# shamim-hussain/tgt

Hardware: AMD Instinct MI355X
Metric: graphs/sec training step, TGT-At 24L PCQM batch 256, 1/2/4/8 MI355X (higher is better)
Workload: dtype bf16

## Files before the change

tgt_amd/csrc/triplet_attention_proj.hip:

```cpp
#include <cstdlib>
#include "triplet_common.hpp"

namespace tgt {

namespace proj2 {
constexpr int kC = xtile::kC, kKS = 16, kRowBytes = xtile::kRowBytes, kSlots = kRowBytes / 16;
constexpr int kXPitch = xtile::kPitch;
constexpr int kXTile = 64 * kXPitch;
constexpr int kSlab = 32 * 8 * 16 * 2;
constexpr int kOffSets = 2 * kXTile, kSet = 3 * kSlab;
constexpr int kOffO = kOffSets + 2 * kSet, kOffBias = kOffO + 2 * kSlab;
constexpr int kLds = kOffBias + 8 * 48 * 4;
constexpr uint32_t kNone = 0xffffffffu;
__device__ __forceinline__ int xoff(int row, int slot) { return xtile::off(row, slot); }
}

__device__ __forceinline__ void zero_o_rows(__amdgpu_buffer_rsrc_t r_out, int tid, int N, uint32_t o_row, uint32_t o_base, uint32_t o_j, int j0) {
    const int srow = (tid & 511) >> 4, sslot = tid & 15;
    const uint32_t vo = (srow < N && tid >= 512) ? (uint32_t)srow * o_row + o_base + (uint32_t)sslot * 16u : proj2::kNone;
    for (int j = j0; j < N; ++j) {
        u32x4_t z = {0, 0, 0, 0};
        __builtin_amdgcn_raw_buffer_store_b128(z, r_out, (int)vo, (int)((uint32_t)j * o_j), TGT_ST_AUX);
    }
}

template <typename T, int DIR, bool STORE, bool RG>
__device__ __forceinline__ void proj2_walk(const tgt_triplet_attention_args& a, const int32_t* node_counts, const TriCtx& c,
                                           const T* x, const T* w, char* smem, int tid) {
    using namespace proj2;
    constexpr int D = 16, HG = 8;
    using G = TriGeo<T, D, HG>;
    using F = frag_t<T>;
    const int lane = tid & 63, wave = tid >> 6, r = lane & 31, hi = lane >> 5;
#ifdef TGT_PROBES
    const uint32_t ablate = a._pad1;
#else
    constexpr uint32_t ablate = 0;
#endif
    const bool attend = wave < 8;
    const int hw = wave & 7;
    const int N = c.N;
    char* xbuf = smem;
    char* sets = smem + kOffSets;
    char* oslab = smem + kOffO;
    const float* bias_w = reinterpret_cast<const float*>(smem + kOffBias) + hw * 48;

    const int64_t sz = sizeof(T), Nl = N;
    const __amdgpu_buffer_rsrc_t r_x = graph_rsrc(x, Nl * Nl * kRowBytes, c.b);
    const uint32_t hch = (uint32_t)(c.g * HG * D * sz), lds_ = (uint32_t)(a.ld_qkv[DIR] * sz), ldo_ = (uint32_t)(a.ld_out * sz);
    const __amdgpu_buffer_rsrc_t r_dst = graph_rsrc(a.qkv[DIR], Nl * Nl * a.ld_qkv[DIR] * sz, c.b);
    const __amdgpu_buffer_rsrc_t r_out = graph_rsrc(a.out, Nl * Nl * a.ld_out * sz, c.b);
    const uint32_t q_row = (uint32_t)N * lds_, q_j = lds_;
    const uint32_t kv_row = DIR == 0 ? lds_ : (uint32_t)N * lds_, kv_j = DIR == 0 ? (uint32_t)N * lds_ : lds_;
    const uint32_t o_row = (uint32_t)N * ldo_, o_j = ldo_;
    auto store_step = [&](int jq, bool qkv_live, int jo, bool o_live) {
        int t_ = tid;
        asm volatile("" : "+v"(t_));
        const int srow = (t_ & 511) >> 4, sslot = t_ & 15, shalf = t_ >> 9;
        const int s_lds = G::lds_off(srow, sslot);
        const bool row_ok = srow < N;
        const uint32_t c16 = (uint32_t)sslot * 16u + hch;
        if constexpr (!STORE) {
            const uint4 vb = *reinterpret_cast<const uint4*>(oslab + (jo & 1) * kSlab + s_lds);
            const uint32_t vo_o = (uint32_t)srow * o_row + (uint32_t)jo * o_j + (uint32_t)(a.o_off[DIR] * sz) + c16;
            u32x4_t db = {vb.x, vb.y, vb.z, vb.w};
            if (ablate & 2) return;
            __builtin_amdgcn_sched_barrier(0);
            __builtin_amdgcn_raw_buffer_store_b128(db, r_out, (int)((row_ok && o_live && shalf == 1) ? vo_o : kNone), 0, TGT_ST_AUX);
            __builtin_amdgcn_sched_barrier(0);
            return;
        }
        const char* set = sets + (jq & 1) * kSet;
        const uint4 va = *reinterpret_cast<const uint4*>(set + shalf * kSlab + s_lds);
        const uint4 vb = *reinterpret_cast<const uint4*>((shalf == 0 ? set + 2 * kSlab : oslab + (jo & 1) * kSlab) + s_lds);
        const uint32_t vo_a = (uint32_t)srow * (shalf == 0 ? q_row : kv_row) + (uint32_t)jq * (shalf == 0 ? q_j : kv_j) +
                              (uint32_t)((shalf == 0 ? a.q_off[DIR] : a.k_off[DIR]) * sz) + c16;
        const uint32_t vo_v = (uint32_t)srow * kv_row + (uint32_t)jq * kv_j + (uint32_t)(a.v_off[DIR] * sz) + c16;
        const uint32_t vo_o = (uint32_t)srow * o_row + (uint32_t)jo * o_j + (uint32_t)(a.o_off[DIR] * sz) + c16;
        u32x4_t da = {va.x, va.y, va.z, va.w}, db = {vb.x, vb.y, vb.z, vb.w};
        if (ablate & 2) return;
        __builtin_amdgcn_sched_barrier(0);
        __builtin_amdgcn_raw_buffer_store_b128(da, r_dst, (int)((row_ok && qkv_live) ? vo_a : kNone), 0, TGT_ST_AUX);
        __builtin_amdgcn_raw_buffer_store_b128(db, r_dst, (int)((row_ok && qkv_live && shalf == 0) ? vo_v : kNone), 0, TGT_ST_AUX);
        __builtin_amdgcn_raw_buffer_store_b128(db, r_out, (int)((row_ok && o_live && shalf == 1) ? vo_o : kNone), 0, TGT_ST_AUX);
        __builtin_amdgcn_sched_barrier(0);
    };

    const int n = tri_node_count<RG>(node_counts, c.b, N);
    if ((a.graph_scale && a.graph_scale[c.b] == 0.f) || (RG && n == 0)) {
        zero_o_rows(r_out, tid, N, o_row, (uint32_t)(a.o_off[DIR] * sz) + hch, o_j, 0);
        return;
    }

    const int l16 = lane & 15, l4 = lane >> 4;
#ifndef TGT_PROJ_PRIO
#define TGT_PROJ_PRIO 1
#endif
    if (TGT_PROJ_PRIO != 0 && __builtin_amdgcn_readfirstlane(wave) >= 8 == (TGT_PROJ_PRIO == 1)) __builtin_amdgcn_s_setprio(1);
    if (attend) {
        float biasM[16], gate[16];
        const ThirdArm ta = tri_third_arm(a, DIR);
        arm_stage_load<T, HG, 1>(ta, c.b, DIR, c.g, N, 0, smem, tid);
        __syncthreads();
        arm_stage_read<T, HG, 1, false>(ta, smem, DIR, hw, N, r, hi, 0, 0, biasM, gate);
        __syncthreads();
        constexpr int kXIt = DIR == 0 ? 4 : 2;
        uint32_t xvo[kXIt];
        int xlo[kXIt];
#pragma unroll
        for (int it = 0; it < kXIt; ++it) {
            const int cidx = it * 512 + tid, row = cidx >> 5, slot = cidx & 31;
            const int node = row & 31;
            xvo[it] = node < N ? (row < 32 ? (uint32_t)node * (uint32_t)N * kRowBytes : (uint32_t)node * kRowBytes) + (uint32_t)slot * 16u : kNone;
            xlo[it] = xoff(row, slot);
        }
        uint4 px[kXIt];
        auto x_issue = [&](int jx) {
            const bool live = jx < n && !(ablate & 1);
#pragma unroll
            for (int it = 0; it < kXIt; ++it) {
                const bool kvrows = DIR == 0 && it >= 2;
                const uint32_t so = live ? (uint32_t)jx * (kvrows ? (uint32_t)N * kRowBytes : (uint32_t)kRowBytes) : 0u;
                const u32x4_t v = __builtin_amdgcn_raw_buffer_load_b128(r_x, (int)(live ? xvo[it] : kNone), (int)so, 0);
                px[it] = make_uint4(v.x, v.y, v.z, v.w);
            }
        };
        auto x_commit = [&](int jx) {
            char* xt = xbuf + (jx & 1) * kXTile;
#pragma unroll
            for (int it = 0; it < kXIt; ++it) *reinterpret_cast<uint4*>(xt + xlo[it]) = px[it];
        };
        F ident_d[1];
        make_ident_d<T, 1>(ident_d, r, hi);
        x_issue(0);
        x_commit(0);
        x_issue(1);
        x_commit(1);
        __syncthreads();
        __syncthreads();
        if constexpr (STORE) store_step(0, true, 0, false);
        for (int j = 0; j < n; ++j) {
            x_issue(j + 2);
            asm volatile("" ::: "memory");
            if (!(ablate & 8)) {
                const char* set = sets + (j & 1) * kSet;
                F fq[1], fk[1], fv[1];
                read_frags<T, D, HG>(fq, set, hw, r, hi);
                read_frags<T, D, HG>(fk, set + kSlab, hw, r, hi);
                read_frags<T, D, HG>(fv, set + 2 * kSlab, hw, r, hi);
                f32x16 z0 = {0}, z1 = {0};
                f32x16 st = mma32(fk[0], fq[0], z0);
                f32x16 vt = mma32(fv[0], ident_d[0], z1);
                float mx = -INFINITY;
#pragma unroll
                for (int q = 0; q < 16; ++q) {
                    st[q] = st[q] * a.scale + biasM[q];
                    mx = fmaxf(mx, st[q]);
                }
                mx = fmaxf(mx, xhalf(mx));
                float sum = 0.f;
#pragma unroll
                for (int q = 0; q < 16; ++q) {
                    st[q] = fast_exp(st[q] - mx);
                    sum += st[q];
                }
                sum += xhalf(sum);
                const float inv = fast_rcp(sum);
#pragma unroll
                for (int q = 0; q < 16; ++q) st[q] = st[q] * inv * gate[q];
                f32x16 o = {0};
#pragma unroll
                for (int cc = 0; cc < 2; ++cc) o = mma32(pack_chunk<T>(vt, cc), pack_chunk<T>(st, cc), o);
                write_rows<T, D, HG>(oslab + (j & 1) * kSlab, o, hw, r, hi);
            }
            x_commit(j + 2);
            __syncthreads();
            if constexpr (STORE) store_step(j + 1, j + 1 < n, j, true);
        }
    } else {
        F wq[kKS / 2], wkv[kKS];
        {
            const T* rq = w + (int64_t)(a.q_off[DIR] + c.h * D + l16) * kC;
            const T* rkv = w + (int64_t)((r < 16 ? a.k_off[DIR] : a.v_off[DIR]) + c.h * D + (r & 15)) * kC;
#pragma unroll
            for (int s2 = 0; s2 < kKS / 2; ++s2) wq[s2] = load_frag<T>(rq + 32 * s2 + 8 * l4);
#pragma unroll
            for (int s2 = 0; s2 < kKS; ++s2) wkv[s2] = load_frag<T>(rkv + 16 * s2 + 8 * hi);
        }
        auto project = [&](int jn) {
            const char* xt = xbuf + (jn & 1) * kXTile;
            char* set = sets + (jn & 1) * kSet;
            constexpr int kv0 = DIR == 0 ? 32 : 0;
            {
                f32x16 kva;
#pragma unroll
                for (int q = 0; q < 16; ++q) kva[q] = bias_w[16 + acc_row(q, hi)];
#pragma unroll
                for (int s2 = 0; s2 < kKS; ++s2) {
                    const F xk = load_frag<T>(reinterpret_cast<const T*>(xt + xoff(kv0 + r, 2 * s2 + hi)));
                    kva = mma32(wkv[s2], xk, kva);
                    if ((s2 & 3) == 3) __builtin_amdgcn_sched_barrier(0);
                }
#pragma unroll
                for (int part = 0; part < 2; ++part)
#pragma unroll
                    for (int q = 0; q < 2; ++q) {
                        T tmp[4];
#pragma unroll
                        for (int t = 0; t < 4; ++t) tmp[t] = from_f32<T>(kva[8 * part + 4 * q + t]);
                        uint2 v;
                        __builtin_memcpy(&v, tmp, 8);
                        *reinterpret_cast<uint2*>(set + (1 + part) * kSlab + G::lds_elem(r, hw * D + 8 * q + 4 * hi)) = v;
                    }
            }
            __builtin_amdgcn_sched_barrier(0);
            {
                f32x4 q0, q1;
#pragma unroll
                for (int t = 0; t < 4; ++t) q0[t] = q1[t] = bias_w[4 * l4 + t];
#pragma unroll
                for (int s2 = 0; s2 < kKS / 2; ++s2) {
                    const F x0 = load_frag<T>(reinterpret_cast<const T*>(xt + xoff(l16, 4 * s2 + l4)));
                    const F x1 = load_frag<T>(reinterpret_cast<const T*>(xt + xoff(16 + l16, 4 * s2 + l4)));
                    q0 = mma16x32(wq[s2], x0, q0);
                    q1 = mma16x32(wq[s2], x1, q1);
                    if (s2 & 1) __builtin_amdgcn_sched_barrier(0);
                }
                T t0[4], t1[4];
#pragma unroll
                for (int t = 0; t < 4; ++t) { t0[t] = from_f32<T>(q0[t]); t1[t] = from_f32<T>(q1[t]); }
                uint2 v0, v1;
                __builtin_memcpy(&v0, t0, 8);
                __builtin_memcpy(&v1, t1, 8);
                *reinterpret_cast<uint2*>(set + G::lds_elem(l16, hw * D + 4 * l4)) = v0;
                *reinterpret_cast<uint2*>(set + G::lds_elem(16 + l16, hw * D + 4 * l4)) = v1;
            }
        };
        __syncthreads();
        __syncthreads();
        __syncthreads();
        project(0);
        __syncthreads();
        if constexpr (STORE) store_step(0, true, 0, false);
        for (int j = 0; j < n; ++j) {
            if (j + 1 < n && !(ablate & 4)) project(j + 1);
            __syncthreads();
            store_step(j + 1, j + 1 < n, j, true);
        }
    }
    if constexpr (RG) {
        int t_ = tid;
        asm volatile("" : "+v"(t_));
        zero_o_rows(r_out, t_, N, o_row, (uint32_t)(a.o_off[DIR] * sz) + hch, o_j, n);
    }
}

template <typename T, bool STORE, typename... NC>
__global__ void __launch_bounds__(1024, 4) tri_att_proj_fwd_kernel(const tgt_triplet_attention_args a, const T* x, const T* w, const T* bias,
                                                                   NC... nc) {
    constexpr bool RG = sizeof...(NC) > 0;
    const int32_t* node_counts = tri_counts_ptr(nc...);
    constexpr int D = 16, HG = 8;
    extern __shared__ __attribute__((aligned(16))) char smem[];
    const int tid = threadIdx.x, lane = tid & 63, wave = tid >> 6;
    const TriCtx c = tri_ctx<T, D, HG>(a, wave & 7);
    const int dir = c.dir;
    if (wave >= 8 && lane < 48) {
        const int part = lane >> 4, d = lane & 15;
        const int off = part == 0 ? a.q_off[dir] : (part == 1 ? a.k_off[dir] : a.v_off[dir]);
        reinterpret_cast<float*>(smem + proj2::kOffBias)[(wave & 7) * 48 + lane] = to_f32(bias[off + c.h * D + d]);
    }
    if (dir == 0) proj2_walk<T, 0, STORE, RG>(a, node_counts, c, x, w, smem, tid);
    else proj2_walk<T, 1, STORE, RG>(a, node_counts, c, x, w, smem, tid);
}

template <typename T>
static int launch_proj(const tgt_triplet_attention_args& a, const int32_t* nc, const void* x, const void* w, const void* bias, hipStream_t st) {
    const int grid = a.B * 2 * (a.H / 8);
    static_assert(ArmStage<T, 8, 1>::kBytes <= proj2::kOffO, "arm stage must fit the aliased area");
#ifdef TGT_PROBES
    static const int ablate = getenv("TGT_PROJ_ABLATE") ? atoi(getenv("TGT_PROJ_ABLATE")) : 0;
    tgt_triplet_attention_args aa = a;
    aa._pad1 = (uint32_t)ablate;
#else
    const tgt_triplet_attention_args& aa = a;
#endif
    const T *xp = reinterpret_cast<const T*>(x), *wp = reinterpret_cast<const T*>(w), *bp = reinterpret_cast<const T*>(bias);
    const dim3 g(grid), blk(1024);
    if (a.flags & TGT_TRI_NO_QKV_STORE)
        return nc ? launch_lds<tri_att_proj_fwd_kernel<T, false, const int32_t*>>("tri_att_proj_fwd_kernel", g, blk, proj2::kLds, st, aa, xp, wp, bp, nc)
                  : launch_lds<tri_att_proj_fwd_kernel<T, false>>("tri_att_proj_fwd_kernel", g, blk, proj2::kLds, st, aa, xp, wp, bp);
    return nc ? launch_lds<tri_att_proj_fwd_kernel<T, true, const int32_t*>>("tri_att_proj_fwd_kernel", g, blk, proj2::kLds, st, aa, xp, wp, bp, nc)
              : launch_lds<tri_att_proj_fwd_kernel<T, true>>("tri_att_proj_fwd_kernel", g, blk, proj2::kLds, st, aa, xp, wp, bp);
}

int triplet_attention_proj_supported(const tgt_triplet_attention_args* a, int C) {
    return a && a->dropout_p == 0.f && a->N <= 32 && a->D == 16 && a->H % 8 == 0 && (a->dtype == TGT_BF16 || a->dtype == TGT_F16) &&
           C == 256;
}

int triplet_attention_proj_run(const tgt_triplet_attention_args* a, const int32_t* nc, const void* x, int C, const void* w,
                               const void* bias, hipStream_t st) {
    if (!a || !x || !w || !bias) return set_error(TGT_ERR_INVALID, "projected triplet attention: null argument");
    if (a->B < 0 || a->N < 0 || a->H <= 0) return set_error(TGT_ERR_INVALID, "projected triplet attention: bad sizes");
    if (a->B == 0 || a->N == 0) return TGT_OK;
    if (!triplet_attention_proj_supported(a, C))
        return set_error(TGT_ERR_UNSUPPORTED,
                         "projected triplet attention needs N <= 32, D = 16, H %% 8 == 0, a 16-bit dtype, C = 256 and no attention dropout "
                         "(got N=%d D=%d H=%d dtype=%d C=%d)", a->N, a->D, a->H, a->dtype, C);
    const bool store = !(a->flags & TGT_TRI_NO_QKV_STORE);
    for (int dir = 0; dir < 2; ++dir) {
        if ((store && !a->qkv[dir]) || !a->out || !a->mask) return set_error(TGT_ERR_INVALID, "projected triplet attention: null tensor");
        if (store && ((a->ld_qkv[dir] * 2) % 16 || (a->q_off[dir] * 2) % 16 || (a->k_off[dir] * 2) % 16 || (a->v_off[dir] * 2) % 16 ||
                      ((uintptr_t)a->qkv[dir] % 16)))
            return set_error(TGT_ERR_INVALID, "projected triplet attention: rows/offsets must be 16-byte aligned");
        if ((a->ld_out * 2) % 16 || (a->o_off[dir] * 2) % 16 || ((uintptr_t)a->out % 16))
            return set_error(TGT_ERR_INVALID, "projected triplet attention: rows/offsets must be 16-byte aligned");
        if ((a->flags & (TGT_TRI_BIASED | TGT_TRI_GATED)) && !a->eg[dir]) return set_error(TGT_ERR_INVALID, "projected triplet attention: eg missing");
    }
    if (((uintptr_t)x | (uintptr_t)w) % 16) return set_error(TGT_ERR_INVALID, "projected triplet attention: x / w must be 16-byte aligned");
    return a->dtype == TGT_BF16 ? launch_proj<bf16_t>(*a, nc, x, w, bias, st) : launch_proj<f16_t>(*a, nc, x, w, bias, st);
}

}
```

Before: 3265.

## Rebalance triplet projection waves: Q-proj on attend waves, direct-to-LDS X loads

Moves the Q projection into the attention waves and leaves only the K/V projection on the projector waves. The projector waves now load X tiles straight into LDS with buffer_load ... lds (m0 set by hand), replacing the register staging and commit step. The X tile layout changes to paired rows with an XOR swizzle. V is read transposed with ds_read_tr16 instead of an identity MFMA, and the default wave priority boost is disabled. This is meant to balance work between the two wave groups and remove VGPR round-trips, at the cost of inline asm fragility and new synchronisation ordering risks.

```diff
diff --git a/tgt_amd/csrc/triplet_attention_proj.hip b/tgt_amd/csrc/triplet_attention_proj.hip
--- a/tgt_amd/csrc/triplet_attention_proj.hip
+++ b/tgt_amd/csrc/triplet_attention_proj.hip
@@ -5,14 +5,27 @@
 
 namespace proj2 {
 constexpr int kC = xtile::kC, kKS = 16, kRowBytes = xtile::kRowBytes, kSlots = kRowBytes / 16;
-constexpr int kXPitch = xtile::kPitch;
-constexpr int kXTile = 64 * kXPitch;
+constexpr int kXPair = 2 * kRowBytes + 32;
+constexpr int kXTile = 32 * kXPair;
+static_assert(kXTile == 64 * xtile::kPitch, "the X tiles keep their size");
 constexpr int kSlab = 32 * 8 * 16 * 2;
 constexpr int kOffSets = 2 * kXTile, kSet = 3 * kSlab;
 constexpr int kOffO = kOffSets + 2 * kSet, kOffBias = kOffO + 2 * kSlab;
 constexpr int kLds = kOffBias + 8 * 48 * 4;
 constexpr uint32_t kNone = 0xffffffffu;
-__device__ __forceinline__ int xoff(int row, int slot) { return xtile::off(row, slot); }
+__device__ __forceinline__ int xoff(int row, int low) { return (row >> 1) * kXPair + (row & 1) * kRowBytes + ((low ^ (row & 1)) << 4); }
+
+typedef short s16x4 __attribute__((ext_vector_type(4)));
+typedef __attribute__((address_space(3))) s16x4 lds_s16x4;
+template <typename T>
+__device__ __forceinline__ frag_t<T> vt_frag(const char* lo, const char* hi) {
+    const s16x4 a = __builtin_amdgcn_ds_read_tr16_b64_v4i16(reinterpret_cast<lds_s16x4*>((uint32_t)(uintptr_t)lo));
+    const s16x4 b = __builtin_amdgcn_ds_read_tr16_b64_v4i16(reinterpret_cast<lds_s16x4*>((uint32_t)(uintptr_t)hi));
+    frag_t<T> f;
+    __builtin_memcpy(&f, &a, 8);
+    __builtin_memcpy(reinterpret_cast<char*>(&f) + 8, &b, 8);
+    return f;
+}
 }
 
 __device__ __forceinline__ void zero_o_rows(__amdgpu_buffer_rsrc_t r_out, int tid, int N, uint32_t o_row, uint32_t o_base, uint32_t o_j, int j0) {
@@ -46,7 +59,6 @@
     const float* bias_w = reinterpret_cast<const float*>(smem + kOffBias) + hw * 48;
 
     const int64_t sz = sizeof(T), Nl = N;
-    const __amdgpu_buffer_rsrc_t r_x = graph_rsrc(x, Nl * Nl * kRowBytes, c.b);
     const uint32_t hch = (uint32_t)(c.g * HG * D * sz), lds_ = (uint32_t)(a.ld_qkv[DIR] * sz), ldo_ = (uint32_t)(a.ld_out * sz);
     const __amdgpu_buffer_rsrc_t r_dst = graph_rsrc(a.qkv[DIR], Nl * Nl * a.ld_qkv[DIR] * sz, c.b);
     const __amdgpu_buffer_rsrc_t r_out = graph_rsrc(a.out, Nl * Nl * a.ld_out * sz, c.b);
@@ -94,7 +106,7 @@
 
     const int l16 = lane & 15, l4 = lane >> 4;
 #ifndef TGT_PROJ_PRIO
-#define TGT_PROJ_PRIO 1
+#define TGT_PROJ_PRIO 0
 #endif
     if (TGT_PROJ_PRIO != 0 && __builtin_amdgcn_readfirstlane(wave) >= 8 == (TGT_PROJ_PRIO == 1)) __builtin_amdgcn_s_setprio(1);
     if (attend) {
@@ -104,146 +116,180 @@
         __syncthreads();
         arm_stage_read<T, HG, 1, false>(ta, smem, DIR, hw, N, r, hi, 0, 0, biasM, gate);
         __syncthreads();
+        const int vt_lo = G::lds_elem(4 * hi + ((lane & 15) >> 2), hw * D + 4 * (lane & 3));
+        const int vt_hi = G::lds_elem(8 + 4 * hi + ((lane & 15) >> 2), hw * D + 4 * (lane & 3));
+        F wq[kKS / 2];
+#pragma unroll
+        for (int q = 0; q < 16; ++q) asm volatile("" : "+v"(biasM[q]), "+v"(gate[q]));
+        __builtin_amdgcn_sched_barrier(0);
+        {
+            const T* rq = w + (int64_t)(a.q_off[DIR] + c.h * D + l16) * kC;
+#pragma unroll
+            for (int s2 = 0; s2 < kKS / 2; ++s2) wq[s2] = load_frag<T>(rq + 32 * s2 + 8 * l4);
+        }
+        auto project_q = [&](int jn) {
+            int ln = lane;
+            asm volatile("" : "+v"(ln));
+            const int q16 = ln & 15, q4 = ln >> 4;
+            const char* xq = xbuf + (jn & 1) * kXTile + xoff(q16, q4);
+            char* set = sets + (jn & 1) * kSet;
+            f32x4 q0, q1;
+#pragma unroll
+            for (int t = 0; t < 4; ++t) q0[t] = q1[t] = bias_w[4 * q4 + t];
+            F xa[2][2];
+            xa[0][0] = load_frag<T>(reinterpret_cast<const T*>(xq));
+            xa[0][1] = load_frag<T>(reinterpret_cast<const T*>(xq + 8 * kXPair));
+#pragma unroll
+            for (int s2 = 0; s2 < kKS / 2; ++s2) {
+                if (s2 + 1 < kKS / 2) {
+                    xa[(s2 + 1) & 1][0] = load_frag<T>(reinterpret_cast<const T*>(xq + 64 * (s2 + 1)));
+                    xa[(s2 + 1) & 1][1] = load_frag<T>(reinterpret_cast<const T*>(xq + 8 * kXPair + 64 * (s2 + 1)));
+                }
+                __builtin_amdgcn_sched_barrier(0);
+                q0 = mma16x32(wq[s2], xa[s2 & 1][0], q0);
+                q1 = mma16x32(wq[s2], xa[s2 & 1][1], q1);
+                __builtin_amdgcn_sched_barrier(0);
+            }
+            T t0[4], t1[4];
+#pragma unroll
+            for (int t = 0; t < 4; ++t) { t0[t] = from_f32<T>(q0[t]); t1[t] = from_f32<T>(q1[t]); }
+            uint2 v0, v1;
+            __builtin_memcpy(&v0, t0, 8);
+            __builtin_memcpy(&v1, t1, 8);
+            *reinterpret_cast<uint2*>(set + G::lds_elem(q16, hw * D + 4 * q4)) = v0;
+            *reinterpret_cast<uint2*>(set + G::lds_elem(16 + q16, hw * D + 4 * q4)) = v1;
+        };
+        __syncthreads();
+        project_q(0);
+        __syncthreads();
+        if constexpr (STORE) store_step(0, true, 0, false);
+        for (int j = 0; j < n; ++j) {
+            if (j + 1 < n && !(ablate & 4)) project_q(j + 1);
+            __builtin_amdgcn_sched_barrier(0);
+            if (!(ablate & 8)) {
+                const char* set = sets + (j & 1) * kSet;
+                F fq[1], fk[1];
+                read_frags<T, D, HG>(fq, set, hw, r, hi);
+                read_frags<T, D, HG>(fk, set + kSlab, hw, r, hi);
+                f32x16 z0 = {0};
+                f32x16 st = mma32(fk[0], fq[0], z0);
+                float mx = -INFINITY;
+#pragma unroll
+                for (int q = 0; q < 16; ++q) {
+                    st[q] = st[q] * a.scale + biasM[q];
+                    mx = fmaxf(mx, st[q]);
+                }
+                mx = fmaxf(mx, xhalf(mx));
+                float sum = 0.f;
+#pragma unroll
+                for (int q = 0; q < 16; ++q) {
+                    st[q] = fast_exp(st[q] - mx);
+                    sum += st[q];
+                }
+                __builtin_amdgcn_sched_barrier(0);
+                F vtf[2];
+#pragma unroll
+                for (int cc = 0; cc < 2; ++cc)
+                    vtf[cc] = vt_frag<T>(set + 2 * kSlab + vt_lo + cc * 16 * G::kRowBytes, set + 2 * kSlab + vt_hi + cc * 16 * G::kRowBytes);
+                __builtin_amdgcn_sched_barrier(0);
+                sum += xhalf(sum);
+                const float inv = fast_rcp(sum);
+#pragma unroll
+                for (int q = 0; q < 16; ++q) st[q] = st[q] * inv * gate[q];
+                f32x16 o = {0};
+#pragma unroll
+                for (int cc = 0; cc < 2; ++cc) o = mma32(vtf[cc], pack_chunk<T>(st, cc), o);
+                write_rows<T, D, HG>(oslab + (j & 1) * kSlab, o, hw, r, hi);
+            }
+            __syncthreads();
+            if constexpr (STORE) store_step(j + 1, j + 1 < n, j, true);
+        }
+    } else {
+        F wkv[kKS];
+        {
+            const T* rkv = w + (int64_t)((r < 16 ? a.k_off[DIR] : a.v_off[DIR]) + c.h * D + (r & 15)) * kC;
+#pragma unroll
+            for (int s2 = 0; s2 < kKS; ++s2) wkv[s2] = load_frag<T>(rkv + 16 * s2 + 8 * hi);
+        }
+        auto project = [&](int jn) {
+            constexpr int kv0 = DIR == 0 ? 32 : 0;
+            const char* xk = xbuf + (jn & 1) * kXTile + xoff(kv0 + r, hi);
+            char* set = sets + (jn & 1) * kSet;
+            f32x16 kva;
+#pragma unroll
+            for (int q = 0; q < 16; ++q) kva[q] = bias_w[16 + acc_row(q, hi)];
+            constexpr int kGrp = 4;
+            F xb[2][kGrp];
+#pragma unroll
+            for (int t = 0; t < kGrp; ++t) xb[0][t] = load_frag<T>(reinterpret_cast<const T*>(xk + 32 * t));
+#pragma unroll
+            for (int g = 0; g < kKS / kGrp; ++g) {
+                if (g + 1 < kKS / kGrp) {
+#pragma unroll
+                    for (int t = 0; t < kGrp; ++t) xb[(g + 1) & 1][t] = load_frag<T>(reinterpret_cast<const T*>(xk + 32 * (kGrp * (g + 1) + t)));
+                }
+                __builtin_amdgcn_sched_barrier(0);
+#pragma unroll
+                for (int t = 0; t < kGrp; ++t) kva = mma32(wkv[kGrp * g + t], xb[g & 1][t], kva);
+                __builtin_amdgcn_sched_barrier(0);
+            }
+#pragma unroll
+            for (int part = 0; part < 2; ++part)
+#pragma unroll
+                for (int q = 0; q < 2; ++q) {
+                    T tmp[4];
+#pragma unroll
+                    for (int t = 0; t < 4; ++t) tmp[t] = from_f32<T>(kva[8 * part + 4 * q + t]);
+                    uint2 v;
+                    __builtin_memcpy(&v, tmp, 8);
+                    *reinterpret_cast<uint2*>(set + (1 + part) * kSlab + G::lds_elem(r, hw * D + 8 * q + 4 * hi)) = v;
+                }
+        };
+        __syncthreads();
+        __syncthreads();
         constexpr int kXIt = DIR == 0 ? 4 : 2;
+        const int wv = __builtin_amdgcn_readfirstlane(wave) & 7;
         uint32_t xvo[kXIt];
-        int xlo[kXIt];
 #pragma unroll
         for (int it = 0; it < kXIt; ++it) {
-            const int cidx = it * 512 + tid, row = cidx >> 5, slot = cidx & 31;
+            const int pair = it * 8 + wv, row = 2 * pair + hi, slot = (lane & 31) ^ hi;
             const int node = row & 31;
             xvo[it] = node < N ? (row < 32 ? (uint32_t)node * (uint32_t)N * kRowBytes : (uint32_t)node * kRowBytes) + (uint32_t)slot * 16u : kNone;
-            xlo[it] = xoff(row, slot);
-        }
-        uint4 px[kXIt];
+            if (node >= N) {
+                const uint4 z = make_uint4(0, 0, 0, 0);
+                *reinterpret_cast<uint4*>(xbuf + pair * kXPair + lane * 16) = z;
+                *reinterpret_cast<uint4*>(xbuf + kXTile + pair * kXPair + lane * 16) = z;
+            }
+        }
+        const uint64_t x_base = (uint64_t)(uintptr_t)x + (uint64_t)c.b * (uint64_t)(Nl * Nl * kRowBytes);
+        const u32x4_t rx4 = {(uint32_t)x_base, (uint32_t)(x_base >> 32) & 0xffffu, (uint32_t)(Nl * Nl * kRowBytes), 0x00020000u};
+        const uint32_t xlds = (uint32_t)(uintptr_t)xbuf + (uint32_t)(wv * kXPair);
         auto x_issue = [&](int jx) {
-            const bool live = jx < n && !(ablate & 1);
-#pragma unroll
-            for (int it = 0; it < kXIt; ++it) {
-                const bool kvrows = DIR == 0 && it >= 2;
-                const uint32_t so = live ? (uint32_t)jx * (kvrows ? (uint32_t)N * kRowBytes : (uint32_t)kRowBytes) : 0u;
-                const u32x4_t v = __builtin_amdgcn_raw_buffer_load_b128(r_x, (int)(live ? xvo[it] : kNone), (int)so, 0);
-                px[it] = make_uint4(v.x, v.y, v.z, v.w);
+            if (jx < n && !(ablate & 1)) {
+#pragma unroll
+                for (int it = 0; it < kXIt; ++it) {
+                    const bool kvrows = DIR == 0 && it >= 2;
+                    const uint32_t so = (uint32_t)jx * (kvrows ? (uint32_t)N * kRowBytes : (uint32_t)kRowBytes);
+                    const uint32_t dst = xlds + (uint32_t)((jx & 1) * kXTile + it * 8 * kXPair);
+                    uint32_t keep;
+                    asm volatile("s_mov_b32 %0, m0\n\ts_mov_b32 m0, %1\n\ts_nop 0\n\tbuffer_load_dwordx4 %2, %3, %4 offen lds\n\ts_mov_b32 m0, %0"
+                                 : "=&s"(keep) : "s"(dst), "v"(xvo[it]), "s"(rx4), "s"(so) : "memory");
+                }
             }
         };
-        auto x_commit = [&](int jx) {
-            char* xt = xbuf + (jx & 1) * kXTile;
-#pragma unroll
-            for (int it = 0; it < kXIt; ++it) *reinterpret_cast<uint4*>(xt + xlo[it]) = px[it];
-        };
-        F ident_d[1];
-        make_ident_d<T, 1>(ident_d, r, hi);
+        auto x_wait = [&]() { asm volatile("s_waitcnt vmcnt(0)" ::: "memory"); };
         x_issue(0);
-        x_commit(0);
         x_issue(1);
-        x_commit(1);
-        __syncthreads();
+        x_wait();
+        __syncthreads();
+        project(0);
         __syncthreads();
         if constexpr (STORE) store_step(0, true, 0, false);
         for (int j = 0; j < n; ++j) {
             x_issue(j + 2);
             asm volatile("" ::: "memory");
-            if (!(ablate & 8)) {
-                const char* set = sets + (j & 1) * kSet;
-                F fq[1], fk[1], fv[1];
-                read_frags<T, D, HG>(fq, set, hw, r, hi);
-                read_frags<T, D, HG>(fk, set + kSlab, hw, r, hi);
-                read_frags<T, D, HG>(fv, set + 2 * kSlab, hw, r, hi);
-                f32x16 z0 = {0}, z1 = {0};
-                f32x16 st = mma32(fk[0], fq[0], z0);
-                f32x16 vt = mma32(fv[0], ident_d[0], z1);
-                float mx = -INFINITY;
-#pragma unroll
-                for (int q = 0; q < 16; ++q) {
-                    st[q] = st[q] * a.scale + biasM[q];
-                    mx = fmaxf(mx, st[q]);
-                }
-                mx = fmaxf(mx, xhalf(mx));
-                float sum = 0.f;
-#pragma unroll
-                for (int q = 0; q < 16; ++q) {
-                    st[q] = fast_exp(st[q] - mx);
-                    sum += st[q];
-                }
-                sum += xhalf(sum);
-                const float inv = fast_rcp(sum);
-#pragma unroll
-                for (int q = 0; q < 16; ++q) st[q] = st[q] * inv * gate[q];
-                f32x16 o = {0};
-#pragma unroll
-                for (int cc = 0; cc < 2; ++cc) o = mma32(pack_chunk<T>(vt, cc), pack_chunk<T>(st, cc), o);
-                write_rows<T, D, HG>(oslab + (j & 1) * kSlab, o, hw, r, hi);
-            }
-            x_commit(j + 2);
-            __syncthreads();
-            if constexpr (STORE) store_step(j + 1, j + 1 < n, j, true);
-        }
-    } else {
-        F wq[kKS / 2], wkv[kKS];
-        {
-            const T* rq = w + (int64_t)(a.q_off[DIR] + c.h * D + l16) * kC;
-            const T* rkv = w + (int64_t)((r < 16 ? a.k_off[DIR] : a.v_off[DIR]) + c.h * D + (r & 15)) * kC;
-#pragma unroll
-            for (int s2 = 0; s2 < kKS / 2; ++s2) wq[s2] = load_frag<T>(rq + 32 * s2 + 8 * l4);
-#pragma unroll
-            for (int s2 = 0; s2 < kKS; ++s2) wkv[s2] = load_frag<T>(rkv + 16 * s2 + 8 * hi);
-        }
-        auto project = [&](int jn) {
-            const char* xt = xbuf + (jn & 1) * kXTile;
-            char* set = sets + (jn & 1) * kSet;
-            constexpr int kv0 = DIR == 0 ? 32 : 0;
-            {
-                f32x16 kva;
-#pragma unroll
-                for (int q = 0; q < 16; ++q) kva[q] = bias_w[16 + acc_row(q, hi)];
-#pragma unroll
-                for (int s2 = 0; s2 < kKS; ++s2) {
-                    const F xk = load_frag<T>(reinterpret_cast<const T*>(xt + xoff(kv0 + r, 2 * s2 + hi)));
-                    kva = mma32(wkv[s2], xk, kva);
-                    if ((s2 & 3) == 3) __builtin_amdgcn_sched_barrier(0);
-                }
-#pragma unroll
-                for (int part = 0; part < 2; ++part)
-#pragma unroll
-                    for (int q = 0; q < 2; ++q) {
-                        T tmp[4];
-#pragma unroll
-                        for (int t = 0; t < 4; ++t) tmp[t] = from_f32<T>(kva[8 * part + 4 * q + t]);
-                        uint2 v;
-                        __builtin_memcpy(&v, tmp, 8);
-                        *reinterpret_cast<uint2*>(set + (1 + part) * kSlab + G::lds_elem(r, hw * D + 8 * q + 4 * hi)) = v;
-                    }
-            }
-            __builtin_amdgcn_sched_barrier(0);
-            {
-                f32x4 q0, q1;
-#pragma unroll
-                for (int t = 0; t < 4; ++t) q0[t] = q1[t] = bias_w[4 * l4 + t];
-#pragma unroll
-                for (int s2 = 0; s2 < kKS / 2; ++s2) {
-                    const F x0 = load_frag<T>(reinterpret_cast<const T*>(xt + xoff(l16, 4 * s2 + l4)));
-                    const F x1 = load_frag<T>(reinterpret_cast<const T*>(xt + xoff(16 + l16, 4 * s2 + l4)));
-                    q0 = mma16x32(wq[s2], x0, q0);
-                    q1 = mma16x32(wq[s2], x1, q1);
-                    if (s2 & 1) __builtin_amdgcn_sched_barrier(0);
-                }
-                T t0[4], t1[4];
-#pragma unroll
-                for (int t = 0; t < 4; ++t) { t0[t] = from_f32<T>(q0[t]); t1[t] = from_f32<T>(q1[t]); }
-                uint2 v0, v1;
-                __builtin_memcpy(&v0, t0, 8);
-                __builtin_memcpy(&v1, t1, 8);
-                *reinterpret_cast<uint2*>(set + G::lds_elem(l16, hw * D + 4 * l4)) = v0;
-                *reinterpret_cast<uint2*>(set + G::lds_elem(16 + l16, hw * D + 4 * l4)) = v1;
-            }
-        };
-        __syncthreads();
-        __syncthreads();
-        __syncthreads();
-        project(0);
-        __syncthreads();
-        if constexpr (STORE) store_step(0, true, 0, false);
-        for (int j = 0; j < n; ++j) {
             if (j + 1 < n && !(ablate & 4)) project(j + 1);
+            x_wait();
             __syncthreads();
             store_step(j + 1, j + 1 < n, j, true);
         }
```

Result: no change. 3280 (median of 6 runs) (+0.5%).
